# zama-ai/verifiable-fhe-paper

Hardware: AMD Instinct MI355X
Metric: vPBS proofs/sec at N=1024 (1/2/4/8 GPU); prover ms/proof vs CPU baseline (higher is better)
Workload: dtype u64; 1 GPU; N=1024 vPBS as IVC chain (BASELINE config 2; verified_pbs ivc_based_vpbs.rs:159-386) via vpbs_ivc_prove_pbs; step = 1 chained proof of the cyclic circuit (2^16 rows) per chain; chains_per_gpu=8, parallelism=replicas, witness=host

## Files before the change

__graft_entry__.py:

```python
import os
import subprocess
import sys

ROOT = os.path.dirname(os.path.abspath(__file__))
for p in (ROOT, os.path.join(ROOT, "tests"), os.path.join(ROOT, "circuitgen")):
    if p not in sys.path:
        sys.path.insert(0, p)


def build():
    import vpbs_amd
    vpbs_amd.build_library()
    subprocess.check_call(["make", "-C", os.path.join(ROOT, "oracle")], stdout=subprocess.DEVNULL)
    vpbs_amd.lib()
    build_example()
    build_example("prove_bsk_hash")
    build_example("prove_step_circuit")
    build_example("prove_ivc")
    build_asm_edge_tool()
    build_product_tool()
    build_reduction_tool()
    build_layer_tool()
    build_fake_rccl()
    sys.path.insert(0, os.path.join(ROOT, "tools"))
    import export_circuits
    export_circuits.ensure_standard()


def build_example(name="prove_step"):
    out = os.path.join(ROOT, "examples", name)
    src = os.path.join(ROOT, "examples", name + ".cpp")
    lib = os.path.join(ROOT, "verifiable-fhe-paper_amd", "libvpbs_hip.so")
    if not os.path.exists(out) or os.path.getmtime(out) < max(os.path.getmtime(src), os.path.getmtime(lib)):
        subprocess.check_call(["g++", "-O2", "-std=c++17", "-pthread", "-I", os.path.join(ROOT, "include"), src, "-L",
                               os.path.join(ROOT, "verifiable-fhe-paper_amd"), "-lvpbs_hip",
                               "-Wl,-rpath,$ORIGIN/../verifiable-fhe-paper_amd", "-Wl,-rpath-link,/opt/rocm/lib", "-o", out])
    return out
# ... 29 lines not shown

def build_reduction_tool():
    out = os.path.join(ROOT, "tools", "test_reductions")
    src = os.path.join(ROOT, "tools", "test_reductions.hip")
    deps = [src] + [os.path.join(ROOT, "verifiable-fhe-paper_amd", "csrc", f) for f in ("gl.h", "poseidon.h")]
    if not os.path.exists(out) or os.path.getmtime(out) < max(os.path.getmtime(d) for d in deps):
        subprocess.check_call(["/opt/rocm/bin/hipcc", "--offload-arch=gfx950", "-O3", "-std=c++17", src, "-o", out])
    return out


def build_layer_tool():
    out = os.path.join(ROOT, "tools", "test_layers")
    src = os.path.join(ROOT, "tools", "test_layers.hip")
    deps = [src] + [os.path.join(ROOT, "verifiable-fhe-paper_amd", "csrc", f)
                    for f in ("gl.h", "poseidon.h", "poseidon_partial_groups.inc", "poseidon_constants.inc")]
    if not os.path.exists(out) or os.path.getmtime(out) < max(os.path.getmtime(d) for d in deps):
        subprocess.check_call(["/opt/rocm/bin/hipcc", "--offload-arch=gfx950", "-O3", "-std=c++17", src, "-o", out])
    return out


def smoke():
    import numpy as np
    import vpbs_amd
    import step_oracle
    from vpbs_amd import synth

    log_n = 10
    ctx = vpbs_amd.Context(0, log_n_max=16)
    inputs = synth.step_inputs(log_n)
    digest = np.array([1, 2, 3, 4], np.uint64)
# ... 116 lines not shown
```

verifiable-fhe-paper_amd/csrc/gates.hip:

```cpp
#include <algorithm>
#include <cstdio>
#include <cstdlib>
#include <cstring>
#include <string>
#include <vector>

#include "context.h"
#include "gates.h"

namespace vpbs {
namespace {
constexpr unsigned THREADS = 256;
struct PiHash {
    u64 h[4];
};

struct DevVars {
    using F = u64;
    const u64* wires;
    const u64* consts;
    size_t stride, j;
    PiHash pih;
    __device__ __forceinline__ u64 wire(unsigned i) const { return wires[(size_t)i * stride + j]; }
    __device__ __forceinline__ u64 constant(unsigned i) const { return consts[(size_t)i * stride + j]; }
    __device__ __forceinline__ u64 pi_hash(unsigned i) const { return pih.h[i]; }
};
using gl::LazyAcc;
template <int NC> struct DevSinkT {
    const u64* row[NC];
    unsigned idx;
    LazyAcc acc[NC];
    __device__ __forceinline__ DevSinkT(const u64* apow, unsigned pow_stride, unsigned nc) : idx(0), acc{} {
#pragma unroll
        for (int a = 0; a < NC; ++a) row[a] = apow + (size_t)((unsigned)a < nc ? (unsigned)a : nc - 1) * pow_stride;
    }
    __device__ __forceinline__ void push(u64 c) {
        const u32 c0 = (u32)c, c1 = (u32)(c >> 32);
#pragma unroll
        for (int a = 0; a < NC; ++a) {
            const u64 p = row[a][idx];
            acc[a].mac(c0, c1, (u32)p, (u32)(p >> 32));
        }
        ++idx;
    }
};

template <class Vars, class DevSink> __device__ __forceinline__ void poseidon_mds_dev(const Vars& v, DevSink& s) {
    u64 a[12], b[12];
#pragma unroll
    for (int i = 0; i < 12; ++i) {
        a[i] = v.wire(2 * i);
        b[i] = v.wire(2 * i + 1);
    }
    poseidon::mds_add_const(a, nullptr);
    poseidon::mds_add_const(b, nullptr);
#pragma unroll
    for (int r = 0; r < 12; ++r) {
        s.push(gl::sub_a(v.wire(24 + 2 * r), a[r]));
        s.push(gl::sub_a(v.wire(25 + 2 * r), b[r]));
    }
}

template <class Vars, class DevSink> __device__ __forceinline__ void poseidon_gate_dev(const Vars& v, DevSink& s) {
    using poseidon::rc;
    const u64 swap = v.wire(24);
    s.push(gl::mul(swap, gl::sub(swap, 1)));
    u64 st[12];
#pragma unroll
    for (int i = 0; i < 4; ++i) {
        const u64 lhs = v.wire(i), rhs = v.wire(i + 4), delta = v.wire(25 + i);
        s.push(gl::sub(gl::mul(swap, gl::sub(rhs, lhs)), delta));
        st[i] = gl::add(lhs, delta);
        st[i + 4] = gl::sub(rhs, delta);
    }
#pragma unroll
    for (int i = 8; i < 12; ++i) st[i] = v.wire(i);
#pragma unroll
    for (int i = 0; i < 12; ++i) st[i] = gl::add_nc(st[i], rc(i));
    for (int r = 0; r < 4; ++r) {
        u64 kc[12];
#pragma unroll
        for (int i = 0; i < 12; ++i) kc[i] = rc(12 * (r + 1) + i);
        if (r != 0) {
#pragma unroll
            for (int i = 0; i < 12; ++i) {
                const u64 in = v.wire(29 + 12 * (r - 1) + i);
                s.push(gl::sub_a(st[i], in));
                st[i] = in;
            }
        }
#pragma unroll
        for (int i = 0; i < 12; i += 2) poseidon::sbox2(st[i], st[i + 1]);
        poseidon::mds_add_const(st, kc);
    }
    for (int g = 0; g < 7; ++g) {
        u64 w[3], x[2];
#pragma unroll
        for (int i = 0; i < 3; ++i) w[i] = v.wire(65 + 3 * g + i);
        s.push(gl::sub_a(st[0], w[0]));
        poseidon::partial_group3_core<true>(st, g, w, x);
        s.push(gl::sub(x[0], w[1]));
        s.push(gl::sub(x[1], w[2]));
    }
    {
        u64 kc[12];
#pragma unroll
        for (int i = 0; i < 12; ++i) kc[i] = rc(12 * 26 + i);
        const u64 in = v.wire(65 + 21);
        s.push(gl::sub_a(st[0], in));
        st[0] = poseidon::sbox(in);
        poseidon::mds_add_const(st, kc);
    }
    for (int r = 0; r < 4; ++r) {
        u64 kc[12];
        const int next = r < 3 ? 12 * (27 + r) : 0;
#pragma unroll
        for (int i = 0; i < 12; ++i) kc[i] = rc(next + i);
#pragma unroll
        for (int i = 0; i < 12; ++i) {
            const u64 in = v.wire(87 + 12 * r + i);
            s.push(gl::sub_a(st[i], in));
            st[i] = in;
        }
#pragma unroll
        for (int i = 0; i < 12; i += 2) poseidon::sbox2(st[i], st[i + 1]);
        poseidon::mds_add_const(st, r < 3 ? kc : nullptr);
    }
#pragma unroll
    for (int i = 0; i < 12; ++i) s.push(gl::sub_a(v.wire(12 + i), st[i]));
}

template <int PART, class Vars, class DevSink> __device__ __forceinline__ void poseidon_gate_part(const Vars& v, DevSink& s) {
    using poseidon::rc;
    u64 st[12];
    if constexpr (PART == 2) {
        s.idx = 0;
        const u64 swap = v.wire(24);
        s.push(gl::mul(swap, gl::sub(swap, 1)));
#pragma unroll
        for (int i = 0; i < 4; ++i) {
            const u64 lhs = v.wire(i), rhs = v.wire(i + 4), delta = v.wire(25 + i);
            s.push(gl::sub(gl::mul(swap, gl::sub(rhs, lhs)), delta));
            st[i] = gl::add(lhs, delta);
            st[i + 4] = gl::sub(rhs, delta);
        }
#pragma unroll
        for (int i = 8; i < 12; ++i) st[i] = v.wire(i);
#pragma unroll
        for (int i = 0; i < 12; ++i) st[i] = gl::add_nc(st[i], rc(i));
        for (int r = 0; r < 3; ++r) {
            u64 kc[12];
#pragma unroll
            for (int i = 0; i < 12; ++i) kc[i] = rc(12 * (r + 1) + i);
#pragma unroll
            for (int i = 0; i < 12; i += 2) poseidon::sbox2(st[i], st[i + 1]);
            poseidon::mds_add_const(st, kc);
#pragma unroll
            for (int i = 0; i < 12; ++i) {
                const u64 in = v.wire(29 + 12 * r + i);
                s.push(gl::sub_a(st[i], in));
                st[i] = in;
            }
        }
    }
    if constexpr (PART == 1) {
        s.idx = 41;
        {
            u64 kc[12];
#pragma unroll
            for (int i = 0; i < 12; ++i) {
                kc[i] = rc(12 * 4 + i);
                st[i] = v.wire(29 + 24 + i);
            }
#pragma unroll
            for (int i = 0; i < 12; i += 2) poseidon::sbox2(st[i], st[i + 1]);
            poseidon::mds_add_const(st, kc);
        }
        for (int g = 0; g < 7; ++g) {
            u64 w[3], x[2];
#pragma unroll
            for (int i = 0; i < 3; ++i) w[i] = v.wire(65 + 3 * g + i);
            s.push(gl::sub_a(st[0], w[0]));
            poseidon::partial_group3_core<true>(st, g, w, x);
            s.push(gl::sub(x[0], w[1]));
            s.push(gl::sub(x[1], w[2]));
        }
        {
            u64 kc[12];
#pragma unroll
            for (int i = 0; i < 12; ++i) kc[i] = rc(12 * 26 + i);
            const u64 in = v.wire(65 + 21);
            s.push(gl::sub_a(st[0], in));
            st[0] = poseidon::sbox(in);
            poseidon::mds_add_const(st, kc);
        }
#pragma unroll
        for (int i = 0; i < 12; ++i) s.push(gl::sub_a(st[i], v.wire(87 + i)));
    }
    if constexpr (PART == 3) {
        s.idx = 75;
        for (int r = 0; r < 4; ++r) {
            u64 kc[12];
            const int next = r < 3 ? 12 * (27 + r) : 0;
#pragma unroll
            for (int i = 0; i < 12; ++i) {
                kc[i] = rc(next + i);
                st[i] = v.wire(87 + 12 * r + i);
            }
#pragma unroll
            for (int i = 0; i < 12; i += 2) poseidon::sbox2(st[i], st[i + 1]);
            poseidon::mds_add_const(st, r < 3 ? kc : nullptr);
            if (r < 3) {
#pragma unroll
                for (int i = 0; i < 12; ++i) s.push(gl::sub_a(st[i], v.wire(87 + 12 * (r + 1) + i)));
            }
        }
#pragma unroll
        for (int i = 0; i < 12; ++i) s.push(gl::sub_a(v.wire(12 + i), st[i]));
    }
}

template <unsigned KIND, class Vars, class DevSink>
__device__ __forceinline__ void eval_kind(const vpbs_gate& g, const gates::CosetTables& t, const Vars& v, DevSink& s) {
    if constexpr (KIND == VPBS_GATE_CONSTANT) gates::eval_constant<u64>(g, v, s);
    if constexpr (KIND == VPBS_GATE_PUBLIC_INPUT) gates::eval_public_input<u64>(g, v, s);
    if constexpr (KIND == VPBS_GATE_ARITHMETIC) gates::eval_arithmetic<u64>(g, v, s);
    if constexpr (KIND == VPBS_GATE_BASE_SUM) gates::eval_base_sum<u64>(g, v, s);
    if constexpr (KIND == VPBS_GATE_POSEIDON) poseidon_gate_dev(v, s);
    if constexpr (KIND == VPBS_GATE_POSEIDON_MDS) poseidon_mds_dev(v, s);
    if constexpr (KIND == VPBS_GATE_ARITHMETIC_EXT) gates::eval_arithmetic_ext<u64>(g, v, s);
    if constexpr (KIND == VPBS_GATE_MUL_EXT) gates::eval_mul_ext<u64>(g, v, s);
    if constexpr (KIND == VPBS_GATE_REDUCING) gates::eval_reducing<u64>(g, v, s);
    if constexpr (KIND == VPBS_GATE_REDUCING_EXT) gates::eval_reducing_ext<u64>(g, v, s);
    if constexpr (KIND == VPBS_GATE_RANDOM_ACCESS) gates::eval_random_access<u64>(g, v, s);
// ... 210 lines not shown
    const u64* wires;
    const u64* constants;
    unsigned n_wires, n_constants;
    const u64* pih;
    gl::Ext wire(unsigned i) const { return i < n_wires ? gl::Ext{wires[2 * i], wires[2 * i + 1]} : gl::ext(0); }
    gl::Ext constant(unsigned i) const { return i < n_constants ? gl::Ext{constants[2 * i], constants[2 * i + 1]} : gl::ext(0); }
    u64 pi_hash(unsigned i) const { return pih[i]; }
};
struct HostSink {
    std::vector<gl::Ext> c;
    void push(gl::Ext x) { c.push_back(x); }
};

}

namespace {
bool launch_gate(hipStream_t s, const u64* wires_lde, const u64* consts_lde, size_t len, const vpbs_gate& g, unsigned num_selectors,
                 const u64* d_apow, unsigned pow_stride, unsigned nc, const PiHash& pih, u64* out, int accumulate) {
#define VPBS_GATE_CASE(K) \
    case K: launch_one<K>(s, wires_lde, consts_lde, len, 0, len, g, num_selectors, d_apow, pow_stride, nc, pih, out, accumulate); return true;
    switch (g.kind) {
        VPBS_GATE_CASE(VPBS_GATE_CONSTANT)
        VPBS_GATE_CASE(VPBS_GATE_PUBLIC_INPUT)
        VPBS_GATE_CASE(VPBS_GATE_ARITHMETIC)
        VPBS_GATE_CASE(VPBS_GATE_BASE_SUM)
        VPBS_GATE_CASE(VPBS_GATE_POSEIDON)
        VPBS_GATE_CASE(VPBS_GATE_POSEIDON_MDS)
        VPBS_GATE_CASE(VPBS_GATE_ARITHMETIC_EXT)
        VPBS_GATE_CASE(VPBS_GATE_MUL_EXT)
        VPBS_GATE_CASE(VPBS_GATE_REDUCING)
// ... 68 lines not shown
        }
        for (unsigned l = 0; l < 3; ++l) lanes->used[l] = used[l];
        if (!lanes->skip_sum && (used[1] || used[2])) {
            const size_t words = (size_t)nc * len;
            hipLaunchKernelGGL(add_lanes_kernel, dim3((unsigned)((words + 255) / 256)), dim3(256), 0, s, d_out, used[1] ? out[1] : (const u64*)nullptr,
                               used[2] ? out[2] : (const u64*)nullptr, words);
        }
    }
}

constexpr double TILE_UNIT_COST = 50;
static double tile_weight(const vpbs_gate& g) {
    switch (g.kind) {
        case VPBS_GATE_ARITHMETIC: return 8.0 * g.p0;
        case VPBS_GATE_BASE_SUM: return 8.0 * g.p0 * (g.p1 - 1);
        case VPBS_GATE_POSEIDON_MDS: return 60;
        case VPBS_GATE_ARITHMETIC_EXT: return 17.0 * g.p0;
        case VPBS_GATE_MUL_EXT: return 13.5 * g.p0;
        case VPBS_GATE_REDUCING: return 10.5 * g.p0;
        case VPBS_GATE_REDUCING_EXT: return 11.7 * g.p0;
        case VPBS_GATE_RANDOM_ACCESS: return 235.0 * g.p1 * (1u << g.p0) / 64;
        case VPBS_GATE_EXPONENTIATION: return 8.0 * g.p0;
        case VPBS_GATE_COSET_INTERPOLATION: return 13.4 * (1u << g.p0);
        default: return 0.5 * g.num_constraints;
    }
}
static bool make_tile_plan(const vpbs_gate* gs, unsigned n_gates, unsigned num_selectors, TilePlan& plan) {
    struct Unit {
        unsigned gate, part;
        double weight;
    };
    std::vector<Unit> units;
    unsigned n_coset = 0, max_consts = 0, n_wires = 0;
    for (unsigned i = 0; i < n_gates; ++i) {
        if (!gs[i].num_constraints) continue;
        max_consts = std::max(max_consts, gs[i].num_constants);
        n_wires = std::max(n_wires, gs[i].num_wires);
        if (gs[i].kind == VPBS_GATE_POSEIDON) {
            units.push_back({i, 1, 510 + TILE_UNIT_COST});
            units.push_back({i, 2, 298 + TILE_UNIT_COST});
            units.push_back({i, 3, 404 + TILE_UNIT_COST});
            continue;
        }
        if (gs[i].kind == VPBS_GATE_COSET_INTERPOLATION) {
            if (n_coset++) return false;
            plan.tables = gates::coset_tables(gs[i].p0);
        }
        units.push_back({i, 0, tile_weight(gs[i]) + TILE_UNIT_COST});
    }
    if (units.empty() || units.size() > TILE_MAX_UNITS || n_wires > 135 || n_wires + num_selectors + max_consts > TILE_MAX_COLS) return false;
    std::sort(units.begin(), units.end(), [](const Unit& a, const Unit& b) { return a.weight > b.weight; });
    std::vector<std::vector<Unit>> bins(TILE_WAVES);
    double load[TILE_WAVES] = {0};
    for (const Unit& u : units) {
        const unsigned b = (unsigned)(std::min_element(load, load + TILE_WAVES) - load);
        bins[b].push_back(u);
// ... 33 lines not shown
unsigned launch_gate_terms_fused(hipStream_t s, const Tuning& tune, const u64* wires_lde, const u64* consts_lde, size_t len, const vpbs_gate* gs,
                                 unsigned n_gates, unsigned num_selectors, const u64 pi_hash[4], const u64* d_apow, unsigned pow_stride, unsigned nc,
                                 u64* d_planes) {
    PiHash pih{{pi_hash[0], pi_hash[1], pi_hash[2], pi_hash[3]}};
    if (tune.gates_tile && len % TILE_PTS == 0) {
        TilePlan tp{};
        if (make_tile_plan(gs, n_gates, num_selectors, tp)) {
            const dim3 grid((unsigned)(len / TILE_PTS)), block(TILE_PTS * TILE_WAVES);
            static const bool trace = getenv("VPBS_TRACE_GATES") != nullptr;
            unsigned long long* prof = nullptr;
            if (trace) {
                (void)hipMalloc(&prof, sizeof(unsigned long long) * TILE_MAX_UNITS);
                (void)hipMemsetAsync(prof, 0, sizeof(unsigned long long) * TILE_MAX_UNITS, s);
            }
            if (nc < 1 || nc > 4) return 0;
#define VPBS_TILE_LAUNCH(NC_) \
    hipLaunchKernelGGL((gate_tile_kernel<NC_>), grid, block, 0, s, wires_lde, consts_lde, len, tp, num_selectors, d_apow, pow_stride, nc, pih, d_planes, prof)
            switch (nc) {
                case 1: VPBS_TILE_LAUNCH(1); break;
                case 2: VPBS_TILE_LAUNCH(2); break;
                case 3: VPBS_TILE_LAUNCH(3); break;
                default: VPBS_TILE_LAUNCH(4); break;
            }
#undef VPBS_TILE_LAUNCH
            if (trace) {
                unsigned long long h[TILE_MAX_UNITS];
                (void)vpbs::stream_sync(s);
                (void)hipMemcpy(h, prof, sizeof h, hipMemcpyDeviceToHost);
                (void)hipFree(prof);
                for (unsigned w = 0; w < TILE_WAVES; ++w) {
                    unsigned long long sum = 0;
                    std::fprintf(stderr, "[gate tile cycles] wave %u:", w);
                    for (unsigned u = tp.wave_first[w]; u < tp.wave_first[w + 1]; ++u) {
                        std::fprintf(stderr, " kind %u part %u %.0f", tp.gates[u].kind, tp.part[u], (double)h[u] / grid.x);
                        sum += h[u];
                    }
                    std::fprintf(stderr, "  total %.0f\n", (double)sum / grid.x);
                }
// ... 4 lines not shown
    return 0;
}

void launch_sum_planes(hipStream_t s, const u64* d_planes, unsigned n_planes, size_t words, u64* d_out) {
    hipLaunchKernelGGL(sum_planes_kernel, dim3((unsigned)((words + 255) / 256)), dim3(256), 0, s, d_planes, n_planes, words, d_out);
}

void validate_gates(const vpbs_gate* gs, unsigned n_gates, unsigned num_selectors, unsigned n_constants_cols, unsigned n_wires) {
    VPBS_REQUIRE(gs && n_gates >= 1 && num_selectors >= 1, "no gates");
    for (unsigned i = 0; i < n_gates; ++i) {
        vpbs_gate g = gs[i];
        VPBS_REQUIRE(derive(g), "unsupported gate parameters");
        VPBS_REQUIRE(g.degree == gs[i].degree && g.num_constraints == gs[i].num_constraints && g.num_wires == gs[i].num_wires,
                     "gate list was not produced by vpbs_gates_layout");
        VPBS_REQUIRE(g.num_wires <= n_wires, "gate needs more wires than the wires batch has");
        VPBS_REQUIRE(gs[i].selector_index < num_selectors && num_selectors + g.num_constants <= n_constants_cols,
                     "selector / gate-constant columns out of range");
        VPBS_REQUIRE(gs[i].group_start <= gs[i].index && gs[i].index < gs[i].group_end && gs[i].group_end - gs[i].group_start <= 16,
                     "bad selector group");
    }
}

void gate_terms_at(const vpbs_gate* gs, unsigned n_gates, unsigned num_selectors, const u64* constants_at, unsigned n_constants,
                   const u64* wires_at, unsigned n_wires, const u64 pi_hash[4], const u64* alphas, unsigned nc, u64* out) {
    unsigned max_c = 0;
    for (unsigned i = 0; i < n_gates; ++i) max_c = std::max(max_c, gs[i].num_constraints);
    std::vector<gl::Ext> total(max_c, gl::ext(0));
    for (unsigned i = 0; i < n_gates; ++i) {
        const vpbs_gate& g = gs[i];
        HostVars v{wires_at, constants_at + 2 * (size_t)num_selectors, n_wires, n_constants - num_selectors, pi_hash};
// ... 61 lines not shown
}

int vpbs_gate_id(const vpbs_gate* g, char* buf, size_t len) {
    if (!g || !buf || !len) return VPBS_ERR_INVALID;
    const std::string id = vpbs::gate_id(*g);
    if (id.empty() || id.size() + 1 > len) return VPBS_ERR_INVALID;
    std::memcpy(buf, id.c_str(), id.size() + 1);
    return (int)id.size();
}

int vpbs_gates_layout(vpbs_gate* gs, unsigned n_gates, unsigned max_degree, unsigned* num_selectors, unsigned* num_gate_constraints) {
    if (!gs || !n_gates || !num_selectors || max_degree < 2) return VPBS_ERR_INVALID;
    std::vector<std::pair<std::string, vpbs_gate>> v;
    for (unsigned i = 0; i < n_gates; ++i) {
        if (!vpbs::derive(gs[i])) return VPBS_ERR_INVALID;
        v.push_back({vpbs::gate_id(gs[i]), gs[i]});
    }
    std::sort(v.begin(), v.end(), [](const auto& a, const auto& b) {
        return a.second.degree != b.second.degree ? a.second.degree < b.second.degree : a.first < b.first;
    });
    for (unsigned i = 1; i < n_gates; ++i)
        if (v[i].first == v[i - 1].first) return VPBS_ERR_INVALID;
    unsigned max_c = 0;
    for (unsigned i = 0; i < n_gates; ++i) {
        gs[i] = v[i].second;
        gs[i].index = i;
        max_c = std::max(max_c, gs[i].num_constraints);
    }
    const unsigned max_gate_degree = gs[n_gates - 1].degree;
    if (max_gate_degree + n_gates - 1 <= max_degree) {
// ... 25 lines not shown

int vpbs_gate_terms_at(const vpbs_gate* gs, unsigned n_gates, unsigned num_selectors, const uint64_t* constants_at, unsigned n_constants,
                       const uint64_t* wires_at, unsigned n_wires, const uint64_t pi_hash[4], const uint64_t* alphas, unsigned nc,
                       uint64_t* out) {
    if (!gs || !n_gates || !constants_at || !wires_at || !pi_hash || !alphas || !out || num_selectors > n_constants || !nc)
        return VPBS_ERR_INVALID;
    try {
        vpbs::validate_gates(gs, n_gates, num_selectors, n_constants, n_wires);
    } catch (const vpbs::DeviceError&) {
        return VPBS_ERR_INVALID;
    }
    vpbs::gate_terms_at(gs, n_gates, num_selectors, constants_at, n_constants, wires_at, n_wires, pi_hash, alphas, nc, out);
    return VPBS_OK;
}

}
```

verifiable-fhe-paper_amd/csrc/gl.h:

```cpp
#pragma once
#include <cstdint>
#include <cstddef>

#if defined(__HIPCC__)
#include <hip/hip_runtime.h>
#define GL_HD __host__ __device__ __forceinline__
#else
#define GL_HD inline
#endif

namespace gl {
using u32 = uint32_t;
using u64 = uint64_t;

constexpr u64 P = 0xFFFFFFFF00000001ull;
constexpr u64 EPS = 0xFFFFFFFFull;
constexpr u64 GENERATOR = 7;
constexpr u64 TWO_ADIC_GENERATOR = 1753635133440165772ull;
constexpr unsigned TWO_ADICITY = 32;

GL_HD u64 canon(u64 x) { return x >= P ? x - P : x; }

GL_HD u64 add(u64 a, u64 b) {
    u64 s = a + b;
// ... 352 lines not shown
            : "+v"(e), "+v"(m), "+v"(h), "+v"(ce), "+v"(cm), "+v"(ch)
            : "v"((u32)c), "v"((u32)(c >> 32)), "v"((u32)a), "v"((u32)(a >> 32))
            : "vcc");
    }
    __device__ __forceinline__ u64 reduce() const {
        const u64 lo = e + (m << 32);
        const u64 t = (m >> 32) + ce + (lo < e ? 1u : 0u);
        const u64 H = h + t;
        const u64 hh = (H >> 32) + cm;
        const u64 top = (u64)ch + (H < t ? 1u : 0u) + (hh >> 32);
        return sub_a(reduce128_asm(lo, (u32)H, (u32)hh), top << 32);
    }
};
#endif

GL_HD u64 mul_2e24(u64 x) {
    const u64 lo = x << 24, hi = x >> 40;
    const u64 t = (hi << 32) - hi;
    u64 r = lo + t;
    if (r < t) r += EPS;
    return canon(r);
}
GL_HD u64 mul_2e48(u64 x) {
    const u64 lo = x << 48, h = x >> 16;
    const u64 h0 = h & EPS, h1 = h >> 32;
    const u64 t = (h0 << 32) - h0;
    u64 r = lo + t;
    if (r < t) r += EPS;
    r = canon(r);
    return sub(r, h1);
// ... 85 lines not shown
```

verifiable-fhe-paper_amd/csrc/kernels.h:

```cpp
#pragma once
#include <hip/hip_runtime.h>
#include "gl.h"
#include "../../include/vpbs_prover.h"

namespace vpbs {
using gl::u32;
using gl::u64;

size_t root_table_words(unsigned log_n);
void launch_root_table(hipStream_t s, u64* roots, unsigned log_n, bool inverse);
void launch_prescale_table(hipStream_t s, u64* table, unsigned log_n, unsigned rate_bits, u64 shift);
size_t lde_table_words(unsigned log_n, unsigned rate_bits);
void launch_lde_table(hipStream_t s, u64* table, unsigned log_n, unsigned rate_bits, u64 shift);
void launch_intt(hipStream_t s, const u64* values, u64* coeffs, u64* scratch, const u64* inv_roots, unsigned ncols,
                 unsigned log_n);
void launch_coset_lde(hipStream_t s, const u64* coeffs, u64* out, const u64* roots, const u64* lde_table, unsigned ncols,
                      unsigned log_n, unsigned rate_bits, unsigned block_first = 0, unsigned n_blocks = 0);
void launch_negacyclic(hipStream_t s, u64* data, const u64* table, unsigned batch, unsigned log_n, bool inverse, u64 ninv);

void launch_partial_products(hipStream_t s, const u64* wires, const u64* sigmas, const u64* roots, unsigned n_routed, unsigned log_n,
                             unsigned max_degree, const u64* d_betas, const u64* d_gammas, unsigned num_challenges, u64* out,
                             u64* scratch, unsigned* d_zero_flag);

void launch_l0_table(hipStream_t s, const u64* roots_big, unsigned log_n, unsigned rate_bits, u64* l0);
// ... 6 lines not shown
void launch_quotient_combine(hipStream_t s, u64* q_local, const u64* g0, const u64* g1, const u64* g2, const u64* apow_last, unsigned log_n,
                             unsigned rate_bits, unsigned nc, size_t leaf_offset, size_t local_len);
void launch_quotient_finish(hipStream_t s, const u64* q_gathered, size_t local_len, const u64* inv_roots_big, const u64* unshift_table,
                            unsigned log_n, unsigned rate_bits, unsigned nc, u64* q_nat, u64* scratch, u64* out_coeffs);

struct Tuning {
    size_t wide_threshold = (size_t)1 << 14;
    size_t fri_leaf_wide_threshold = (size_t)1 << 14;
    bool merkle_climb = true;
    bool gates_fused = true;
    unsigned gate_items = 5;
    bool gates_tile = true;
    static Tuning from_env();
};

struct GateLanes {
    hipStream_t stream[2];
    hipEvent_t fork, join[2];
    u64* out[2];
    void (*extra)(hipStream_t, void*) = nullptr;
    void* extra_arg = nullptr;
    unsigned extra_weight = 0;
    bool skip_sum = false;
    bool used[3] = {false, false, false};
};
void launch_gate_terms(hipStream_t s, const u64* wires_lde, const u64* consts_lde, size_t len, const vpbs_gate* gates, unsigned n_gates,
                       unsigned num_selectors, const u64 pi_hash[4], const u64* d_apow, unsigned pow_stride, unsigned nc, u64* d_out,
                       GateLanes* lanes = nullptr);
unsigned gate_terms_planes(const vpbs_gate* gates, unsigned n_gates, unsigned num_selectors, const Tuning& tune, size_t len);
unsigned launch_gate_terms_fused(hipStream_t s, const Tuning& tune, const u64* wires_lde, const u64* consts_lde, size_t len, const vpbs_gate* gates, unsigned n_gates,
// ... 61 lines not shown
```

verifiable-fhe-paper_amd/csrc/prover.hip:

```cpp
#include <algorithm>
#include <cstdio>
#include <cstdlib>

#include "host/plonky2_mirror.h"
#include "proof_shape.h"
#include "witness_check.h"

using vpbs::DeviceError;
using vpbs::Timed;
using vpbs::u32;
using vpbs::u64;

namespace plonky2 {

size_t fri_proof_words(const FriParams& p, const std::vector<size_t>& ncols) {
    if (p.why_invalid(ncols.size())) return 0;
    const unsigned log_lde = p.lde_bits();
    const size_t cap = (size_t)4 << p.config.cap_height;
    size_t w = p.reduction_arity_bits.size() * cap;
    size_t per_q = 0;
    for (size_t nc : ncols) per_q += nc + 4 * (size_t)(log_lde - p.config.cap_height);
    unsigned lg = log_lde;
    for (unsigned ab : p.reduction_arity_bits) {
        lg -= ab;
// ... 299 lines not shown
        ctx->release(scratch);
        throw;
    }
    ctx->release(d_ch);
    ctx->release(scratch);
    VPBS_REQUIRE(flag == 0, "zero denominator in the permutation argument (the reference's batch inverse would panic)");
}


void gate_terms_device(vpbs_ctx* ctx, vpbs_batch* cs, vpbs_batch* wires, const vpbs_gate* gs, unsigned n_gates, unsigned num_selectors,
                       const u64 pi_hash[4], const u64* alphas, unsigned nc, u64* d_out) {
    VPBS_REQUIRE(cs && wires && cs->ctx == ctx && wires->ctx == ctx, "batches of another context");
    VPBS_REQUIRE(cs->log_n == wires->log_n && cs->n_shards == wires->n_shards && cs->shard == wires->shard, "gate terms: batches differ in shape");
    VPBS_REQUIRE(nc >= 1 && nc <= 4, "unsupported number of challenges");
    vpbs::validate_gates(gs, n_gates, num_selectors, cs->ncols, wires->ncols);
    unsigned stride = 1;
    for (unsigned i = 0; i < n_gates; ++i) stride = std::max(stride, gs[i].num_constraints);
    std::vector<u64> h_apow((size_t)nc * stride);
    for (unsigned a = 0; a < nc; ++a) {
        u64 p = 1;
        for (unsigned i = 0; i < stride; ++i) {
            h_apow[(size_t)a * stride + i] = p;
            p = gl::mul(p, alphas[a]);
        }
    }
    u64* d_apow = ctx->alloc_words(h_apow.size());
    const bool multi = ctx->gate_lanes == 3;
    const size_t len = wires->lde_len();
    u64* lane_buf = nullptr;
    const unsigned n_planes = ctx->tune.gates_fused ? vpbs::gate_terms_planes(gs, n_gates, num_selectors, ctx->tune, len) : 0;
    if (n_planes) {
        u64* planes = nullptr;
        try {
            planes = ctx->alloc_words((size_t)n_planes * nc * len);
            VPBS_HIP(hipMemcpyAsync(d_apow, h_apow.data(), sizeof(u64) * h_apow.size(), hipMemcpyHostToDevice, ctx->stream));
            Timed t(ctx, "gate_constraints");
            vpbs::launch_gate_terms_fused(ctx->stream, ctx->tune, wires->d_lde, cs->d_lde, len, gs, n_gates, num_selectors, pi_hash, d_apow, stride, nc, planes);
            vpbs::launch_sum_planes(ctx->stream, planes, n_planes, (size_t)nc * len, d_out);
            VPBS_HIP(hipGetLastError());
        } catch (...) {
// ... 80 lines not shown
    }
    u64* d_apow = ctx->alloc_words(h_apow.size());
    u64* q_leaf = ctx->alloc_words((size_t)nc * big);
    u64* q_nat = ctx->alloc_words((size_t)nc * big);
    u64 *d_gpow = nullptr, *lane_buf = nullptr;
    const size_t local_len = wires->lde_len(), leaf_offset = wires->leaf_offset();
    try {
        VPBS_HIP(hipMemcpyAsync(d_apow, h_apow.data(), sizeof(u64) * h_apow.size(), hipMemcpyHostToDevice, s));
        const u64* l0 = ctx->l0_table(log_n);
        const u64* gathered = q_leaf;
        u64* q_local = world > 1 ? comm->d_stage_local : q_leaf;
        if (world > 1) VPBS_REQUIRE((size_t)nc * local_len <= comm->stage_capacity_words, "comm staging buffers too small for the quotient values");
        if (gw) {
            vpbs::validate_gates(gw->gates, gw->n_gates, gw->num_selectors, cs->ncols, wires->ncols);
            VPBS_REQUIRE(gw->num_selectors <= n_constants, "selector columns must be leading constants columns");
            unsigned stride = 1;
            for (unsigned i = 0; i < gw->n_gates; ++i) stride = std::max(stride, gw->gates[i].num_constraints);
            std::vector<u64> h_gpow((size_t)nc * stride);
            for (unsigned a = 0; a < nc; ++a) {
                u64 p = 1;
                for (unsigned i = 0; i < stride; ++i) {
                    h_gpow[(size_t)a * stride + i] = p;
                    p = gl::mul(p, alphas[a]);
                }
            }
            d_gpow = ctx->alloc_words(h_gpow.size());
            const unsigned n_planes = ctx->tune.gates_fused ? vpbs::gate_terms_planes(gw->gates, gw->n_gates, gw->num_selectors, ctx->tune, local_len) : 0;
            lane_buf = ctx->alloc_words(std::max(3u, n_planes) * (size_t)nc * local_len);
            VPBS_HIP(hipMemcpyAsync(d_gpow, h_gpow.data(), sizeof(u64) * h_gpow.size(), hipMemcpyHostToDevice, s));
            ctx->ensure_gate_lanes();
            u64 apow_last[4] = {0, 0, 0, 0};
            for (unsigned a = 0; a < nc; ++a) apow_last[a] = h_apow[(size_t)a * (n_terms + 1) + n_terms];
            if (n_planes) {
                Timed t(ctx, "gate_constraints");
                VPBS_HIP(hipEventRecord(ctx->gate_fork, s));
                VPBS_HIP(hipStreamWaitEvent(ctx->gate_streams[0], ctx->gate_fork, 0));
                vpbs::launch_quotient_values(ctx->gate_streams[0], wires->d_lde, cs->d_lde + (size_t)n_constants * local_len, zs_pp->d_lde,
                                             ctx->roots(log_big, false), l0, nullptr, d_apow, betas, gammas, n_routed, log_n, rate_bits, max_degree, nc,
                                             leaf_offset, local_len, q_local, true);
                VPBS_HIP(hipEventRecord(ctx->gate_join[0], ctx->gate_streams[0]));
// ... 567 lines not shown
```

Baseline: 0.2300 vPBS proofs/s.

## Fold Poseidon gate linear layers into host-precomputed per-challenge coefficient tables

Poseidon gate constraint evaluation no longer recomputes the MDS and round-constant linear layers per row. The host derives the linear map from S-box inputs and outputs to every constraint and folds it with the alpha powers into one coefficient table per challenge. The device then only computes S-boxes and accumulates products against that table. Accumulation switches to a 22-bit three-limb form with scalar operands so each product is six v_mad_u64_u32. This adds host-side matrix work and a larger table per call, and caps the product count per gate.

Measured after the change: 0.2342 vPBS proofs/s (median of 6 runs). +1.8%, better.

```diff
diff --git a/__graft_entry__.py b/__graft_entry__.py
--- a/__graft_entry__.py
+++ b/__graft_entry__.py
@@ -21,6 +21,7 @@
     build_product_tool()
     build_reduction_tool()
     build_layer_tool()
+    build_limb_acc_tool()
     build_fake_rccl()
     sys.path.insert(0, os.path.join(ROOT, "tools"))
     import export_circuits
@@ -80,6 +81,15 @@
     src = os.path.join(ROOT, "tools", "test_layers.hip")
     deps = [src] + [os.path.join(ROOT, "verifiable-fhe-paper_amd", "csrc", f)
                     for f in ("gl.h", "poseidon.h", "poseidon_partial_groups.inc", "poseidon_constants.inc")]
+    if not os.path.exists(out) or os.path.getmtime(out) < max(os.path.getmtime(d) for d in deps):
+        subprocess.check_call(["/opt/rocm/bin/hipcc", "--offload-arch=gfx950", "-O3", "-std=c++17", src, "-o", out])
+    return out
+
+
+def build_limb_acc_tool():
+    out = os.path.join(ROOT, "tools", "test_limb_acc")
+    src = os.path.join(ROOT, "tools", "test_limb_acc.hip")
+    deps = [src, os.path.join(ROOT, "verifiable-fhe-paper_amd", "csrc", "gl.h")]
     if not os.path.exists(out) or os.path.getmtime(out) < max(os.path.getmtime(d) for d in deps):
         subprocess.check_call(["/opt/rocm/bin/hipcc", "--offload-arch=gfx950", "-O3", "-std=c++17", src, "-o", out])
     return out
diff --git a/verifiable-fhe-paper_amd/csrc/gates.hip b/verifiable-fhe-paper_amd/csrc/gates.hip
--- a/verifiable-fhe-paper_amd/csrc/gates.hip
+++ b/verifiable-fhe-paper_amd/csrc/gates.hip
@@ -1,4 +1,5 @@
 #include <algorithm>
+#include <array>
 #include <cstdio>
 #include <cstdlib>
 #include <cstring>
@@ -7,6 +8,7 @@
 
 #include "context.h"
 #include "gates.h"
+#include "test_entries.h"
 
 namespace vpbs {
 namespace {
@@ -25,118 +27,55 @@
     __device__ __forceinline__ u64 constant(unsigned i) const { return consts[(size_t)i * stride + j]; }
     __device__ __forceinline__ u64 pi_hash(unsigned i) const { return pih.h[i]; }
 };
-using gl::LazyAcc;
+constexpr unsigned FOLD_PB = 0;
+constexpr unsigned FOLD_PW = FOLD_PB + 118;
+constexpr unsigned FOLD_PK = FOLD_PW + 106;
+constexpr unsigned FOLD_MI = FOLD_PK + 1;
+constexpr unsigned FOLD_POW = FOLD_MI + 24;
 template <int NC> struct DevSinkT {
-    const u64* row[NC];
+    const gl::Limbs* row[NC];
     unsigned idx;
-    LazyAcc acc[NC];
+    gl::LimbAcc acc[NC];
     __device__ __forceinline__ DevSinkT(const u64* apow, unsigned pow_stride, unsigned nc) : idx(0), acc{} {
 #pragma unroll
-        for (int a = 0; a < NC; ++a) row[a] = apow + (size_t)((unsigned)a < nc ? (unsigned)a : nc - 1) * pow_stride;
-    }
-    __device__ __forceinline__ void push(u64 c) {
+        for (int a = 0; a < NC; ++a)
+            row[a] = reinterpret_cast<const gl::Limbs*>(apow + (size_t)((unsigned)a < nc ? (unsigned)a : nc - 1) * pow_stride);
+    }
+    __device__ __forceinline__ void mac_at(u64 c, unsigned at) {
         const u32 c0 = (u32)c, c1 = (u32)(c >> 32);
 #pragma unroll
         for (int a = 0; a < NC; ++a) {
-            const u64 p = row[a][idx];
-            acc[a].mac(c0, c1, (u32)p, (u32)(p >> 32));
-        }
-        ++idx;
-    }
+            const gl::Limbs p = row[a][at];
+            acc[a].mac(c0, c1, p.l0, p.l1, p.l2);
+        }
+    }
+    __device__ __forceinline__ void push(u64 c) { mac_at(c, FOLD_POW + idx++); }
 };
 
 template <class Vars, class DevSink> __device__ __forceinline__ void poseidon_mds_dev(const Vars& v, DevSink& s) {
-    u64 a[12], b[12];
-#pragma unroll
-    for (int i = 0; i < 12; ++i) {
-        a[i] = v.wire(2 * i);
-        b[i] = v.wire(2 * i + 1);
-    }
-    poseidon::mds_add_const(a, nullptr);
-    poseidon::mds_add_const(b, nullptr);
-#pragma unroll
-    for (int r = 0; r < 12; ++r) {
-        s.push(gl::sub_a(v.wire(24 + 2 * r), a[r]));
-        s.push(gl::sub_a(v.wire(25 + 2 * r), b[r]));
-    }
-}
-
-template <class Vars, class DevSink> __device__ __forceinline__ void poseidon_gate_dev(const Vars& v, DevSink& s) {
-    using poseidon::rc;
-    const u64 swap = v.wire(24);
-    s.push(gl::mul(swap, gl::sub(swap, 1)));
-    u64 st[12];
-#pragma unroll
-    for (int i = 0; i < 4; ++i) {
-        const u64 lhs = v.wire(i), rhs = v.wire(i + 4), delta = v.wire(25 + i);
-        s.push(gl::sub(gl::mul(swap, gl::sub(rhs, lhs)), delta));
-        st[i] = gl::add(lhs, delta);
-        st[i + 4] = gl::sub(rhs, delta);
-    }
-#pragma unroll
-    for (int i = 8; i < 12; ++i) st[i] = v.wire(i);
-#pragma unroll
-    for (int i = 0; i < 12; ++i) st[i] = gl::add_nc(st[i], rc(i));
-    for (int r = 0; r < 4; ++r) {
-        u64 kc[12];
-#pragma unroll
-        for (int i = 0; i < 12; ++i) kc[i] = rc(12 * (r + 1) + i);
-        if (r != 0) {
-#pragma unroll
-            for (int i = 0; i < 12; ++i) {
-                const u64 in = v.wire(29 + 12 * (r - 1) + i);
-                s.push(gl::sub_a(st[i], in));
-                st[i] = in;
-            }
-        }
-#pragma unroll
-        for (int i = 0; i < 12; i += 2) poseidon::sbox2(st[i], st[i + 1]);
-        poseidon::mds_add_const(st, kc);
-    }
-    for (int g = 0; g < 7; ++g) {
-        u64 w[3], x[2];
-#pragma unroll
-        for (int i = 0; i < 3; ++i) w[i] = v.wire(65 + 3 * g + i);
-        s.push(gl::sub_a(st[0], w[0]));
-        poseidon::partial_group3_core<true>(st, g, w, x);
-        s.push(gl::sub(x[0], w[1]));
-        s.push(gl::sub(x[1], w[2]));
-    }
-    {
-        u64 kc[12];
-#pragma unroll
-        for (int i = 0; i < 12; ++i) kc[i] = rc(12 * 26 + i);
-        const u64 in = v.wire(65 + 21);
-        s.push(gl::sub_a(st[0], in));
-        st[0] = poseidon::sbox(in);
-        poseidon::mds_add_const(st, kc);
-    }
-    for (int r = 0; r < 4; ++r) {
-        u64 kc[12];
-        const int next = r < 3 ? 12 * (27 + r) : 0;
-#pragma unroll
-        for (int i = 0; i < 12; ++i) kc[i] = rc(next + i);
-#pragma unroll
-        for (int i = 0; i < 12; ++i) {
-            const u64 in = v.wire(87 + 12 * r + i);
-            s.push(gl::sub_a(st[i], in));
-            st[i] = in;
-        }
-#pragma unroll
-        for (int i = 0; i < 12; i += 2) poseidon::sbox2(st[i], st[i + 1]);
-        poseidon::mds_add_const(st, r < 3 ? kc : nullptr);
-    }
-#pragma unroll
-    for (int i = 0; i < 12; ++i) s.push(gl::sub_a(v.wire(12 + i), st[i]));
-}
-
-template <int PART, class Vars, class DevSink> __device__ __forceinline__ void poseidon_gate_part(const Vars& v, DevSink& s) {
-    using poseidon::rc;
-    u64 st[12];
-    if constexpr (PART == 2) {
+#pragma unroll
+    for (unsigned j = 0; j < 24; ++j) s.mac_at(v.wire(j), FOLD_MI + j);
+#pragma unroll
+    for (unsigned j = 0; j < 24; ++j) s.push(v.wire(24 + j));
+}
+
+template <class Vars, class DevSink> __device__ __forceinline__ void poseidon_fold_pair(const Vars& v, DevSink& s, unsigned w) {
+    u64 x0 = v.wire(w), x1 = v.wire(w + 1);
+    s.mac_at(x0, FOLD_PW + w - 29);
+    s.mac_at(x1, FOLD_PW + w - 28);
+    poseidon::sbox2(x0, x1);
+    s.mac_at(x0, FOLD_PB + w - 17);
+    s.mac_at(x1, FOLD_PB + w - 16);
+}
+template <bool HEAD, unsigned W0, unsigned W1, bool OUT, class Vars, class DevSink>
+__device__ __forceinline__ void poseidon_gate_fold(const Vars& v, DevSink& s) {
+    static_assert(W0 >= 29 && W1 <= 135 && W0 <= W1 && (W1 - W0) % 2 == 0, "S-box wires in pairs");
+    if constexpr (HEAD) {
+        using poseidon::rc;
         s.idx = 0;
         const u64 swap = v.wire(24);
         s.push(gl::mul(swap, gl::sub(swap, 1)));
+        u64 st[12];
 #pragma unroll
         for (int i = 0; i < 4; ++i) {
             const u64 lhs = v.wire(i), rhs = v.wire(i + 4), delta = v.wire(25 + i);
@@ -148,76 +87,31 @@
         for (int i = 8; i < 12; ++i) st[i] = v.wire(i);
 #pragma unroll
         for (int i = 0; i < 12; ++i) st[i] = gl::add_nc(st[i], rc(i));
-        for (int r = 0; r < 3; ++r) {
-            u64 kc[12];
-#pragma unroll
-            for (int i = 0; i < 12; ++i) kc[i] = rc(12 * (r + 1) + i);
-#pragma unroll
-            for (int i = 0; i < 12; i += 2) poseidon::sbox2(st[i], st[i + 1]);
-            poseidon::mds_add_const(st, kc);
-#pragma unroll
-            for (int i = 0; i < 12; ++i) {
-                const u64 in = v.wire(29 + 12 * r + i);
-                s.push(gl::sub_a(st[i], in));
-                st[i] = in;
-            }
-        }
-    }
-    if constexpr (PART == 1) {
-        s.idx = 41;
-        {
-            u64 kc[12];
-#pragma unroll
-            for (int i = 0; i < 12; ++i) {
-                kc[i] = rc(12 * 4 + i);
-                st[i] = v.wire(29 + 24 + i);
-            }
-#pragma unroll
-            for (int i = 0; i < 12; i += 2) poseidon::sbox2(st[i], st[i + 1]);
-            poseidon::mds_add_const(st, kc);
-        }
-        for (int g = 0; g < 7; ++g) {
-            u64 w[3], x[2];
-#pragma unroll
-            for (int i = 0; i < 3; ++i) w[i] = v.wire(65 + 3 * g + i);
-            s.push(gl::sub_a(st[0], w[0]));
-            poseidon::partial_group3_core<true>(st, g, w, x);
-            s.push(gl::sub(x[0], w[1]));
-            s.push(gl::sub(x[1], w[2]));
-        }
-        {
-            u64 kc[12];
-#pragma unroll
-            for (int i = 0; i < 12; ++i) kc[i] = rc(12 * 26 + i);
-            const u64 in = v.wire(65 + 21);
-            s.push(gl::sub_a(st[0], in));
-            st[0] = poseidon::sbox(in);
-            poseidon::mds_add_const(st, kc);
-        }
-#pragma unroll
-        for (int i = 0; i < 12; ++i) s.push(gl::sub_a(st[i], v.wire(87 + i)));
-    }
-    if constexpr (PART == 3) {
-        s.idx = 75;
-        for (int r = 0; r < 4; ++r) {
-            u64 kc[12];
-            const int next = r < 3 ? 12 * (27 + r) : 0;
-#pragma unroll
-            for (int i = 0; i < 12; ++i) {
-                kc[i] = rc(next + i);
-                st[i] = v.wire(87 + 12 * r + i);
-            }
-#pragma unroll
-            for (int i = 0; i < 12; i += 2) poseidon::sbox2(st[i], st[i + 1]);
-            poseidon::mds_add_const(st, r < 3 ? kc : nullptr);
-            if (r < 3) {
-#pragma unroll
-                for (int i = 0; i < 12; ++i) s.push(gl::sub_a(st[i], v.wire(87 + 12 * (r + 1) + i)));
-            }
-        }
-#pragma unroll
-        for (int i = 0; i < 12; ++i) s.push(gl::sub_a(v.wire(12 + i), st[i]));
-    }
+#pragma unroll
+        for (int i = 0; i < 12; i += 2) poseidon::sbox2(st[i], st[i + 1]);
+#pragma unroll
+        for (int i = 0; i < 12; ++i) s.mac_at(st[i], FOLD_PB + i);
+        s.mac_at(1, FOLD_PK);
+    }
+    constexpr unsigned W4 = W0 + (W1 - W0) / 4 * 4;
+    for (unsigned w = W0; w < W4; w += 4) {
+        poseidon_fold_pair(v, s, w);
+        poseidon_fold_pair(v, s, w + 2);
+    }
+    if constexpr (W4 < W1) poseidon_fold_pair(v, s, W4);
+    if constexpr (OUT) {
+        s.idx = 111;
+#pragma unroll
+        for (int i = 0; i < 12; ++i) s.push(v.wire(12 + i));
+    }
+}
+template <class Vars, class DevSink> __device__ __forceinline__ void poseidon_gate_dev(const Vars& v, DevSink& s) {
+    poseidon_gate_fold<true, 29, 135, true>(v, s);
+}
+template <int PART, class Vars, class DevSink> __device__ __forceinline__ void poseidon_gate_part(const Vars& v, DevSink& s) {
+    if constexpr (PART == 1) poseidon_gate_fold<false, 29, 69, false>(v, s);
+    if constexpr (PART == 2) poseidon_gate_fold<true, 69, 95, false>(v, s);
+    if constexpr (PART == 3) poseidon_gate_fold<false, 95, 135, true>(v, s);
 }
 
 template <unsigned KIND, class Vars, class DevSink>
@@ -458,6 +352,136 @@
 
 }
 
+namespace fold {
+constexpr unsigned N_SBOX = 118, N_VAR = N_SBOX + 1, N_CON = 123;
+struct Matrix {
+    u64 L[N_CON][N_VAR];
+    unsigned lo[N_CON], hi[N_CON];
+    u64 mds[12][12];
+};
+static void derive(Matrix& m) {
+    std::memset(&m, 0, sizeof m);
+    std::vector<std::array<u64, N_VAR>> st(12);
+    unsigned s = 0, idx = 5;
+    auto take = [&](unsigned i) {
+        st[i].fill(0);
+        st[i][s++] = 1;
+    };
+    auto constrain = [&](unsigned i) { std::memcpy(m.L[idx++], st[i].data(), sizeof(u64) * N_VAR); };
+    auto layer = [&](int next_round) {
+        for (unsigned k = 0; k < N_VAR; ++k) {
+            u64 col[12];
+            for (unsigned i = 0; i < 12; ++i) col[i] = st[i][k];
+            gates::Pos<u64>::mds_then_constants(col, k == N_SBOX ? next_round : -1);
+            for (unsigned i = 0; i < 12; ++i) st[i][k] = col[i];
+        }
+    };
+    int round = 0;
+    for (unsigned r = 0; r < 4; ++r, ++round) {
+        for (unsigned i = 0; i < 12; ++i) {
+            if (r != 0) constrain(i);
+            take(i);
+        }
+        layer(round + 1);
+    }
+    for (unsigned r = 0; r < 22; ++r, ++round) {
+        constrain(0);
+        take(0);
+        layer(round + 1);
+    }
+    for (unsigned r = 0; r < 4; ++r, ++round) {
+        for (unsigned i = 0; i < 12; ++i) {
+            constrain(i);
+            take(i);
+        }
+        layer(round + 1 < 30 ? round + 1 : -1);
+    }
+    for (unsigned i = 0; i < 12; ++i) constrain(i);
+    VPBS_REQUIRE(s == N_SBOX && idx == N_CON, "fold matrix: S-box / constraint count");
+    for (idx = 5; idx < N_CON; ++idx) {
+        unsigned lo = N_SBOX, hi = 0;
+        for (unsigned k = 0; k < N_SBOX; ++k)
+            if (m.L[idx][k]) {
+                lo = std::min(lo, k);
+                hi = k + 1;
+            }
+        m.lo[idx] = std::min(lo, hi);
+        m.hi[idx] = hi;
+    }
+    for (unsigned j = 0; j < 12; ++j) {
+        u64 col[12] = {0};
+        col[j] = 1;
+        gates::Pos<u64>::mds_then_constants(col, -1);
+        for (unsigned r = 0; r < 12; ++r) m.mds[r][j] = col[r];
+    }
+}
+static const Matrix& matrix() {
+    static const Matrix* m = [] {
+        Matrix* p = new Matrix;
+        derive(*p);
+        return p;
+    }();
+    return *m;
+}
+static void row(bool poseidon, bool poseidon_mds, u64 alpha, unsigned n_pow, u64* out) {
+    std::fill(out, out + FOLD_POW, 0);
+    u64* pow = out + FOLD_POW;
+    u64 p = 1;
+    for (unsigned i = 0; i < n_pow; ++i) {
+        pow[i] = p;
+        p = gl::mul(p, alpha);
+    }
+    if (poseidon) {
+        VPBS_REQUIRE(n_pow >= N_CON, "gate sink table: fewer powers than the PoseidonGate has constraints");
+        const Matrix& m = matrix();
+        u64 k = 0;
+        for (unsigned idx = 5; idx < N_CON; ++idx) {
+            const u64 a = idx < 111 ? pow[idx] : gl::neg(pow[idx]);
+            for (unsigned s = m.lo[idx]; s < m.hi[idx]; ++s) out[FOLD_PB + s] = gl::add(out[FOLD_PB + s], gl::mul(a, m.L[idx][s]));
+            k = gl::add(k, gl::mul(a, m.L[idx][N_SBOX]));
+            if (idx < 111) out[FOLD_PW + idx - 5] = gl::neg(pow[idx]);
+        }
+        out[FOLD_PK] = k;
+    }
+    if (poseidon_mds) {
+        VPBS_REQUIRE(n_pow >= 24, "gate sink table: fewer powers than the PoseidonMdsGate has constraints");
+        const Matrix& m = matrix();
+        for (unsigned j = 0; j < 12; ++j)
+            for (unsigned c = 0; c < 2; ++c) {
+                u64 t = 0;
+                for (unsigned r = 0; r < 12; ++r) t = gl::add(t, gl::mul(pow[2 * r + c], m.mds[r][j]));
+                out[FOLD_MI + 2 * j + c] = gl::neg(t);
+            }
+    }
+}
+}
+
+static_assert(sizeof(gl::Limbs) == 2 * sizeof(u64), "a table entry is two words");
+size_t gate_sink_row_words(unsigned n_pow) { return 2 * (FOLD_POW + (size_t)n_pow); }
+void gate_sink_table(const vpbs_gate* gs, unsigned n_gates, const u64* alphas, unsigned nc, unsigned n_pow, u64* out) {
+    bool poseidon = false, poseidon_mds = false;
+    for (unsigned i = 0; i < n_gates; ++i) {
+        poseidon |= gs[i].kind == VPBS_GATE_POSEIDON;
+        poseidon_mds |= gs[i].kind == VPBS_GATE_POSEIDON_MDS;
+    }
+    const size_t entries = FOLD_POW + (size_t)n_pow;
+    std::vector<u64> values(entries);
+    for (unsigned a = 0; a < nc; ++a) {
+        fold::row(poseidon, poseidon_mds, alphas[a], n_pow, values.data());
+        for (size_t i = 0; i < entries; ++i) {
+            const gl::Limbs l = gl::limbs(values[i]);
+            std::memcpy(out + 2 * (a * entries + i), &l, sizeof l);
+        }
+    }
+}
+unsigned sink_products(const vpbs_gate& g) {
+    switch (g.kind) {
+        case VPBS_GATE_POSEIDON: return 5 + 12 + 1 + 2 * 106 + 12;
+        case VPBS_GATE_POSEIDON_MDS: return 48;
+        default: return g.num_constraints;
+    }
+}
+
 namespace {
 bool launch_gate(hipStream_t s, const u64* wires_lde, const u64* consts_lde, size_t len, const vpbs_gate& g, unsigned num_selectors,
                  const u64* d_apow, unsigned pow_stride, unsigned nc, const PiHash& pih, u64* out, int accumulate) {
@@ -556,7 +580,7 @@
     switch (g.kind) {
         case VPBS_GATE_ARITHMETIC: return 8.0 * g.p0;
         case VPBS_GATE_BASE_SUM: return 8.0 * g.p0 * (g.p1 - 1);
-        case VPBS_GATE_POSEIDON_MDS: return 60;
+        case VPBS_GATE_POSEIDON_MDS: return 42;
         case VPBS_GATE_ARITHMETIC_EXT: return 17.0 * g.p0;
         case VPBS_GATE_MUL_EXT: return 13.5 * g.p0;
         case VPBS_GATE_REDUCING: return 10.5 * g.p0;
@@ -579,9 +603,9 @@
         max_consts = std::max(max_consts, gs[i].num_constants);
         n_wires = std::max(n_wires, gs[i].num_wires);
         if (gs[i].kind == VPBS_GATE_POSEIDON) {
-            units.push_back({i, 1, 510 + TILE_UNIT_COST});
-            units.push_back({i, 2, 298 + TILE_UNIT_COST});
-            units.push_back({i, 3, 404 + TILE_UNIT_COST});
+            units.push_back({i, 1, 238 + TILE_UNIT_COST});
+            units.push_back({i, 2, 232 + TILE_UNIT_COST});
+            units.push_back({i, 3, 252 + TILE_UNIT_COST});
             continue;
         }
         if (gs[i].kind == VPBS_GATE_COSET_INTERPOLATION) {
@@ -645,14 +669,13 @@
                 (void)hipMemsetAsync(prof, 0, sizeof(unsigned long long) * TILE_MAX_UNITS, s);
             }
             if (nc < 1 || nc > 4) return 0;
-#define VPBS_TILE_LAUNCH(NC_) \
-    hipLaunchKernelGGL((gate_tile_kernel<NC_>), grid, block, 0, s, wires_lde, consts_lde, len, tp, num_selectors, d_apow, pow_stride, nc, pih, d_planes, prof)
-            switch (nc) {
-                case 1: VPBS_TILE_LAUNCH(1); break;
-                case 2: VPBS_TILE_LAUNCH(2); break;
-                case 3: VPBS_TILE_LAUNCH(3); break;
-                default: VPBS_TILE_LAUNCH(4); break;
-            }
+#define VPBS_TILE_LAUNCH(NC_, FIRST_) \
+    hipLaunchKernelGGL((gate_tile_kernel<NC_>), grid, block, 0, s, wires_lde, consts_lde, len, tp, num_selectors, d_apow + (size_t)(FIRST_) * pow_stride, \
+                       pow_stride, (unsigned)(NC_), pih, d_planes + (size_t)(FIRST_) * len, prof)
+            if (nc == 1) VPBS_TILE_LAUNCH(1, 0);
+            else VPBS_TILE_LAUNCH(2, 0);
+            if (nc == 3) VPBS_TILE_LAUNCH(1, 2);
+            if (nc == 4) VPBS_TILE_LAUNCH(2, 2);
 #undef VPBS_TILE_LAUNCH
             if (trace) {
                 unsigned long long h[TILE_MAX_UNITS];
@@ -687,6 +710,7 @@
         VPBS_REQUIRE(g.degree == gs[i].degree && g.num_constraints == gs[i].num_constraints && g.num_wires == gs[i].num_wires,
                      "gate list was not produced by vpbs_gates_layout");
         VPBS_REQUIRE(g.num_wires <= n_wires, "gate needs more wires than the wires batch has");
+        VPBS_REQUIRE(sink_products(g) <= gl::LimbAcc::MAX_PRODUCTS, "gate pushes more products than the device sink's sums hold");
         VPBS_REQUIRE(gs[i].selector_index < num_selectors && num_selectors + g.num_constants <= n_constants_cols,
                      "selector / gate-constant columns out of range");
         VPBS_REQUIRE(gs[i].group_start <= gs[i].index && gs[i].index < gs[i].group_end && gs[i].group_end - gs[i].group_start <= 16,
@@ -778,6 +802,7 @@
     std::vector<std::pair<std::string, vpbs_gate>> v;
     for (unsigned i = 0; i < n_gates; ++i) {
         if (!vpbs::derive(gs[i])) return VPBS_ERR_INVALID;
+        if (vpbs::sink_products(gs[i]) > gl::LimbAcc::MAX_PRODUCTS) return VPBS_ERR_INVALID;
         v.push_back({vpbs::gate_id(gs[i]), gs[i]});
     }
     std::sort(v.begin(), v.end(), [](const auto& a, const auto& b) {
@@ -833,4 +858,78 @@
     return VPBS_OK;
 }
 
-}
+int vpbs_test_gate_fold(unsigned kind, const uint64_t* alphas, unsigned nc, const uint64_t* wires, size_t n, uint64_t* direct, uint64_t* folded) {
+    using namespace vpbs;
+    if (!alphas || !wires || !direct || !folded || !nc || !n || (kind != VPBS_GATE_POSEIDON && kind != VPBS_GATE_POSEIDON_MDS)) return VPBS_ERR_INVALID;
+    struct RowVars {
+        const u64* w;
+        u64 wire(unsigned i) const { return w[i]; }
+        u64 constant(unsigned) const { return 0; }
+        u64 pi_hash(unsigned) const { return 0; }
+    };
+    struct PowerSink {
+        u64 alpha, pow = 1, sum = 0;
+        void push(u64 c) {
+            sum = gl::add(sum, gl::mul(pow, c));
+            pow = gl::mul(pow, alpha);
+        }
+    };
+    struct RowSink {
+        const u64* row;
+        unsigned idx = 0;
+        u64 sum = 0;
+        void mac_at(u64 c, unsigned at) {
+            gl::Limbs l;
+            std::memcpy(&l, row + 2 * at, sizeof l);
+            sum = gl::add(sum, gl::mul(c, gl::unlimbs(l)));
+        }
+        void push(u64 c) { mac_at(c, FOLD_POW + idx++); }
+    };
+    vpbs_gate g{};
+    g.kind = kind;
+    if (!derive(g)) return VPBS_ERR_INVALID;
+    const unsigned n_pow = g.num_constraints, stride = (unsigned)gate_sink_row_words(n_pow);
+    std::vector<u64> table((size_t)nc * stride);
+    try {
+        gate_sink_table(&g, 1, alphas, nc, n_pow, table.data());
+    } catch (const DeviceError&) {
+        return VPBS_ERR_INVALID;
+    }
+    for (size_t j = 0; j < n; ++j) {
+        const RowVars v{wires + j * g.num_wires};
+        for (unsigned a = 0; a < nc; ++a) {
+            PowerSink d{alphas[a]};
+            RowSink s{table.data() + (size_t)a * stride};
+            if (kind == VPBS_GATE_POSEIDON_MDS) {
+                gates::eval_poseidon_mds<u64>(g, v, d);
+                for (unsigned k = 0; k < 24; ++k) s.mac_at(v.wire(k), FOLD_MI + k);
+                for (unsigned k = 0; k < 24; ++k) s.push(v.wire(24 + k));
+            } else {
+                gates::eval_poseidon<u64>(g, v, d);
+                const u64 swap = v.wire(24);
+                s.push(gl::mul(swap, gl::sub(swap, 1)));
+                u64 st[12];
+                for (unsigned i = 0; i < 4; ++i) {
+                    const u64 lhs = v.wire(i), rhs = v.wire(i + 4), delta = v.wire(25 + i);
+                    s.push(gl::sub(gl::mul(swap, gl::sub(rhs, lhs)), delta));
+                    st[i] = gl::add(lhs, delta);
+                    st[i + 4] = gl::sub(rhs, delta);
+                }
+                for (unsigned i = 8; i < 12; ++i) st[i] = v.wire(i);
+                for (unsigned i = 0; i < 12; ++i) s.mac_at(gates::Pos<u64>::sbox(gl::add(st[i], poseidon::rc(i))), FOLD_PB + i);
+                s.mac_at(1, FOLD_PK);
+                for (unsigned w = 29; w < 135; ++w) {
+                    s.mac_at(v.wire(w), FOLD_PW + w - 29);
+                    s.mac_at(gates::Pos<u64>::sbox(v.wire(w)), FOLD_PB + w - 17);
+                }
+                s.idx = 111;
+                for (unsigned i = 0; i < 12; ++i) s.push(v.wire(12 + i));
+            }
+            direct[j * nc + a] = d.sum;
+            folded[j * nc + a] = s.sum;
+        }
+    }
+    return VPBS_OK;
+}
+
+}
diff --git a/verifiable-fhe-paper_amd/csrc/gl.h b/verifiable-fhe-paper_amd/csrc/gl.h
--- a/verifiable-fhe-paper_amd/csrc/gl.h
+++ b/verifiable-fhe-paper_amd/csrc/gl.h
@@ -390,6 +390,42 @@
 };
 #endif
 
+struct alignas(16) Limbs {
+    u32 l0, l1, l2, pad;
+};
+GL_HD Limbs limbs(u64 a) { return Limbs{(u32)(a & 0x3fffffu), (u32)((a >> 22) & 0x3fffffu), (u32)(a >> 44), 0}; }
+GL_HD u64 unlimbs(Limbs l) { return (u64)l.l0 | ((u64)l.l1 << 22) | ((u64)l.l2 << 44); }
+struct LimbAcc {
+    static constexpr unsigned MAX_PRODUCTS = 1024;
+    u64 s[6];
+    GL_HD void mac(u32 c0, u32 c1, u32 l0, u32 l1, u32 l2) {
+#if defined(__HIP_DEVICE_COMPILE__)
+        asm("v_mad_u64_u32 %0, vcc, %6, %8, %0\n\t"
+            "v_mad_u64_u32 %1, vcc, %6, %9, %1\n\t"
+            "v_mad_u64_u32 %2, vcc, %6, %10, %2\n\t"
+            "v_mad_u64_u32 %3, vcc, %7, %8, %3\n\t"
+            "v_mad_u64_u32 %4, vcc, %7, %9, %4\n\t"
+            "v_mad_u64_u32 %5, vcc, %7, %10, %5"
+            : "+v"(s[0]), "+v"(s[1]), "+v"(s[2]), "+v"(s[3]), "+v"(s[4]), "+v"(s[5])
+            : "v"(c0), "v"(c1), "s"(l0), "s"(l1), "s"(l2)
+            : "vcc");
+#else
+        s[0] += (u64)c0 * l0;
+        s[1] += (u64)c0 * l1;
+        s[2] += (u64)c0 * l2;
+        s[3] += (u64)c1 * l0;
+        s[4] += (u64)c1 * l1;
+        s[5] += (u64)c1 * l2;
+#endif
+    }
+    GL_HD u64 reduce() const {
+        using u128 = unsigned __int128;
+        const u128 U = (u128)s[0] + ((u128)s[1] << 22) + ((u128)s[2] << 44) + ((u128)s[3] << 32) + ((u128)s[4] << 54) + ((u128)(s[5] & 0xfffffu) << 76);
+        const u64 hi = (u64)(U >> 64);
+        return sub_a(reduce128_asm((u64)U, (u32)hi, (u32)(hi >> 32)), s[5] >> 20);
+    }
+};
+
 GL_HD u64 mul_2e24(u64 x) {
     const u64 lo = x << 24, hi = x >> 40;
     const u64 t = (hi << 32) - hi;
diff --git a/verifiable-fhe-paper_amd/csrc/kernels.h b/verifiable-fhe-paper_amd/csrc/kernels.h
--- a/verifiable-fhe-paper_amd/csrc/kernels.h
+++ b/verifiable-fhe-paper_amd/csrc/kernels.h
@@ -44,6 +44,8 @@
     static Tuning from_env();
 };
 
+size_t gate_sink_row_words(unsigned n_pow);
+void gate_sink_table(const vpbs_gate* gates, unsigned n_gates, const u64* alphas, unsigned nc, unsigned n_pow, u64* out);
 struct GateLanes {
     hipStream_t stream[2];
     hipEvent_t fork, join[2];
diff --git a/verifiable-fhe-paper_amd/csrc/prover.hip b/verifiable-fhe-paper_amd/csrc/prover.hip
--- a/verifiable-fhe-paper_amd/csrc/prover.hip
+++ b/verifiable-fhe-paper_amd/csrc/prover.hip
@@ -337,16 +337,11 @@
     VPBS_REQUIRE(cs->log_n == wires->log_n && cs->n_shards == wires->n_shards && cs->shard == wires->shard, "gate terms: batches differ in shape");
     VPBS_REQUIRE(nc >= 1 && nc <= 4, "unsupported number of challenges");
     vpbs::validate_gates(gs, n_gates, num_selectors, cs->ncols, wires->ncols);
-    unsigned stride = 1;
-    for (unsigned i = 0; i < n_gates; ++i) stride = std::max(stride, gs[i].num_constraints);
+    unsigned n_pow = 1;
+    for (unsigned i = 0; i < n_gates; ++i) n_pow = std::max(n_pow, gs[i].num_constraints);
+    const unsigned stride = (unsigned)vpbs::gate_sink_row_words(n_pow);
     std::vector<u64> h_apow((size_t)nc * stride);
-    for (unsigned a = 0; a < nc; ++a) {
-        u64 p = 1;
-        for (unsigned i = 0; i < stride; ++i) {
-            h_apow[(size_t)a * stride + i] = p;
-            p = gl::mul(p, alphas[a]);
-        }
-    }
+    vpbs::gate_sink_table(gs, n_gates, alphas, nc, n_pow, h_apow.data());
     u64* d_apow = ctx->alloc_words(h_apow.size());
     const bool multi = ctx->gate_lanes == 3;
     const size_t len = wires->lde_len();
@@ -457,16 +452,11 @@
         if (gw) {
             vpbs::validate_gates(gw->gates, gw->n_gates, gw->num_selectors, cs->ncols, wires->ncols);
             VPBS_REQUIRE(gw->num_selectors <= n_constants, "selector columns must be leading constants columns");
-            unsigned stride = 1;
-            for (unsigned i = 0; i < gw->n_gates; ++i) stride = std::max(stride, gw->gates[i].num_constraints);
+            unsigned n_pow = 1;
+            for (unsigned i = 0; i < gw->n_gates; ++i) n_pow = std::max(n_pow, gw->gates[i].num_constraints);
+            const unsigned stride = (unsigned)vpbs::gate_sink_row_words(n_pow);
             std::vector<u64> h_gpow((size_t)nc * stride);
-            for (unsigned a = 0; a < nc; ++a) {
-                u64 p = 1;
-                for (unsigned i = 0; i < stride; ++i) {
-                    h_gpow[(size_t)a * stride + i] = p;
-                    p = gl::mul(p, alphas[a]);
-                }
-            }
+            vpbs::gate_sink_table(gw->gates, gw->n_gates, alphas, nc, n_pow, h_gpow.data());
             d_gpow = ctx->alloc_words(h_gpow.size());
             const unsigned n_planes = ctx->tune.gates_fused ? vpbs::gate_terms_planes(gw->gates, gw->n_gates, gw->num_selectors, ctx->tune, local_len) : 0;
             lane_buf = ctx->alloc_words(std::max(3u, n_planes) * (size_t)nc * local_len);
```
